# yjpark1/multiagent_rl

Hardware: AMD Instinct MI355X
Metric: env-steps/sec, simple_spread N=6 x B envs, 1/2/4/8 MI355X (higher is better)
Workload: dtype f32

## Files before the change

multiagent_rl_amd/csrc/pw_kernels_spread_quad.hpp:

```cpp
#pragma once

#include "pw_kernels_spread.hpp"

namespace {

__device__ __forceinline__ void quad_pair_of(const int q, int &i, int &j)
{
    i = q < 5 ? 0 : q < 9 ? 1 : q < 12 ? 2 : q < 14 ? 3 : 4;
    j = q - (i == 0 ? 0 : i == 1 ? 5 : i == 2 ? 9 : i == 3 ? 12 : 14) + i + 1;
}

#ifndef PW_QUAD_BARRIER
#define PW_QUAD_BARRIER(t) duo_barrier()
#endif
#ifndef PW_QUAD_ACT_AHEAD
#define PW_QUAD_ACT_AHEAD 4
#endif
constexpr int kQuadActAhead = PW_QUAD_ACT_AHEAD;
constexpr int kQuadActRingBytes = kQuadActAhead * kWave * (int)sizeof(int32_t);
template <bool UNIT_MASS, bool COLL = false, bool K1 = false>
__global__ void __launch_bounds__(4 * kWave) pw_spread_quad_kernel(const StreamParams A, const int T)
{
    constexpr int N = 6, L = 6, D = 16, P2 = 15, EPP = 4, EPW = 8;
    extern __shared__ __attribute__((aligned(16))) unsigned char smem_raw[];
    float4 *s_ring = reinterpret_cast<float4 *>(smem_raw);
    float2 *s_ftab = reinterpret_cast<float2 *>(s_ring + 4 * kWave);
    float *s_min = reinterpret_cast<float *>(s_ftab + 2 * EPP * N * N);
    float *s_rew = s_min + kWave;
    float2 *s_lmB = reinterpret_cast<float2 *>(s_rew + kWave);
    int32_t *s_act = reinterpret_cast<int32_t *>(s_lmB + EPW * L);
    float2 *s_utab = reinterpret_cast<float2 *>(s_act + 2 * kQuadActAhead * kWave);

    const int wave = __builtin_amdgcn_readfirstlane((((int)threadIdx.x >> 6) + 2 * (((int)blockIdx.x >> 8) & 1)) & 3);
    const int lane = (int)threadIdx.x & 63;
    const int env0 = (int)blockIdx.x * EPW;
    const int envs_here = A.B - env0 < EPW ? A.B - env0 : EPW;
    const size_t BN = (size_t)A.B * N;

    const bool resets = A.auto_reset && A.max_episode_len > 0;
    int offs_all = A.ep_step[env0 + (lane < envs_here ? lane : 0)];
    auto next_reset_step = [&](int t_from) -> int {
        if (!resets) return 0x7fffffff;
        int rem = A.max_episode_len - 1 - (t_from + offs_all);
        rem = rem < 0 ? 0 : rem;
        int m = 0x7fffffff;
        for (int e = 0; e < envs_here; ++e) {
            const int r = __builtin_amdgcn_readlane(rem, e);
            m = r < m ? r : m;
        }
        return t_from + m;
    };
    int t_reset = next_reset_step(0);
    auto reset_step_update = [&](int t) {
        if (t + 1 + offs_all >= A.max_episode_len) offs_all = -(t + 1);
        t_reset = next_reset_step(t + 1);
    };
    int cur = 0;

    if (wave < 2) {
        __builtin_amdgcn_s_setprio(3);
        const int e0 = wave * EPP;
        const int nv = envs_here - e0 < 0 ? 0 : envs_here - e0 < EPP ? envs_here - e0 : EPP;
        if (nv == 0) {
            for (int t = 0; t < T; ++t) PW_QUAD_BARRIER(t);
            return;
        }
        const int la = lane < nv * N ? lane : 0;
        const int e4 = la / N, a = la - e4 * N;
        const int me = (e0 + e4) * N + a;
        const int env = env0 + e0 + e4;
        const uint32_t g = (uint32_t)env * (uint32_t)N + (uint32_t)a;
        const uint64_t env_id = A.env_id_base + (uint64_t)env;
        const int lp = lane < nv * P2 ? lane : 0;
        const int pe = lp / P2, pq = lp - pe * P2;
        int pi, pj;
        quad_pair_of(pq, pi, pj);
        const int ri = (e0 + pe) * N + pi, rj = (e0 + pe) * N + pj;
        float2 *ftab = s_ftab + wave * (EPP * N * N);
        float2 *f_ij = ftab + (pe * N + pi) * N + (pj - 1), *f_ji = ftab + (pe * N + pj) * N + pi;
        const float2 *row = ftab + (e4 * N + a) * N;

        float px = A.pos_x[g], py = A.pos_y[g], vx = A.vel_x[g], vy = A.vel_y[g];
        int ep_off = A.ep_step[env];
        uint32_t ep_count = A.ep_count[env];
        s_ring[me] = make_float4(px, py, vx, vy);
        float2 *utab = s_utab + wave * 8;
        if (lane < 6) {
            const int ai = lane;
            float ux = 0.0f + ((ai == 1 ? 1.0f : 0.0f) - (ai == 2 ? 1.0f : 0.0f));
            float uy = 0.0f + ((ai == 3 ? 1.0f : 0.0f) - (ai == 4 ? 1.0f : 0.0f));
            ux *= A.sens; uy *= A.sens;
            if (A.fscale != 1.0f) { ux = A.fscale * ux; uy = A.fscale * uy; }
            utab[lane] = make_float2(ux + 0.0f, uy + 0.0f);
        }
        wave_lds_sync();
        const float k = A.contact_margin, cf = A.contact_force, dt = A.dt, damp = A.damp, mass = A.mass;
        const uint32_t near_lo = __float_as_uint(A.near_thr2), near_span = 0x7F800000u - near_lo;
        const int32_t *act_g = A.act + g;
        int32_t *act_ring = s_act + wave * (kQuadActAhead * kWave);
        const uint32_t act_lds = __builtin_amdgcn_readfirstlane((uint32_t)reinterpret_cast<uintptr_t>(act_ring));
        auto fetch_act = [&](int t) {
            act_fetch_issue(act_g + (size_t)(t < T ? t : T - 1) * BN, act_lds + (uint32_t)(t & (kQuadActAhead - 1)) * (kWave * 4));
        };
        asm volatile("" :: "v"(ep_off), "v"(ep_count), "v"(offs_all), "v"(px), "v"(py), "v"(vx), "v"(vy), "s"(t_reset));
        for (int t0 = 0; t0 < kQuadActAhead; ++t0) fetch_act(t0);
        float2 qi = *reinterpret_cast<const float2 *>(s_ring + ri);
        float2 qj = *reinterpret_cast<const float2 *>(s_ring + rj);
        PW_STAMP_DECL;
        for (int t = 0; t < T; ++t) {
            PW_STAMP_START;
            asm volatile("s_waitcnt vmcnt(%0)" :: "n"(kQuadActAhead - 1) : "memory");
            PW_STAMP(3);
            const uint32_t ai = (uint32_t)act_ring[(t & (kQuadActAhead - 1)) * kWave + lane];
            fetch_act(t + kQuadActAhead);
            const float2 u0 = utab[ai < 5u ? ai : 5u];
            const bool two_slots = t == t_reset;
            float Fx = 0.0f, Fy = 0.0f;
            {
                const float dx = qi.x - qj.x, dy = qi.y - qj.y;
                const float d2 = dx * dx + dy * dy;
                if (__float_as_uint(d2) - near_lo >= near_span)
                    collision_force_pair<true, K1>(qi.x, qi.y, qj.x, qj.y, A.dist_min, k, cf, Fx, Fy);
            }
            *f_ij = make_float2(Fx, Fy);
            *f_ji = make_float2(-Fx, -Fy);
            PW_STAMP(0);
            float fx = u0.x, fy = u0.y;
            asm volatile("" ::: "memory");
#pragma unroll
            for (int j = 0; j < N - 1; ++j) {
                const float2 F = row[j];
                fx = F.x + fx;
                fy = F.y + fy;
            }
            vx = vx * damp; vy = vy * damp;
            vx = vx + div_mass<UNIT_MASS>(fx, mass) * dt;
            vy = vy + div_mass<UNIT_MASS>(fy, mass) * dt;
            px = px + vx * dt;
            py = py + vy * dt;
            int nxt = (cur + 1) & 3;
            s_ring[nxt * kWave + me] = make_float4(px, py, vx, vy);
            if (two_slots) {
                if (t + 1 + ep_off >= A.max_episode_len) {
                    ep_count += 1;
                    ep_off = -(t + 1);
                    pw_reset_xy(A.seed, env_id, ep_count, (uint32_t)a, -1.0f, 1.0f, &px, &py);
                    vx = 0.f; vy = 0.f;
                }
                reset_step_update(t);
                nxt = (nxt + 1) & 3;
                s_ring[nxt * kWave + me] = make_float4(px, py, vx, vy);
            }
            cur = nxt;
            asm volatile("" ::: "memory");
            qi = *reinterpret_cast<const float2 *>(s_ring + cur * kWave + ri);
            qj = *reinterpret_cast<const float2 *>(s_ring + cur * kWave + rj);
            PW_STAMP(1);
            PW_QUAD_BARRIER(t);
            PW_STAMP(2);
        }
        act_fetch_drain();
#ifdef PW_STAMPS
        if (blockIdx.x == 0 && wave == 0 && lane == 0)
            for (int i_ = 0; i_ < 4; ++i_) g_pw_stamps[i_] = st_acc[i_];
#endif
        A.pos_x[g] = px; A.pos_y[g] = py;
        A.vel_x[g] = vx; A.vel_y[g] = vy;
        A.ep_step[env] = T + ep_off;
        A.ep_count[env] = ep_count;
        return;
    }

    int e_local = lane / N;
    int a = lane - e_local * N;
    if (e_local >= envs_here) { e_local = 0; a = 0; }
    const int env = env0 + e_local;
    const int base = e_local * N, me = base + a;
    const uint32_t g = (uint32_t)env * (uint32_t)N + (uint32_t)a;
    const uint64_t env_id = A.env_id_base + (uint64_t)env;
    int ep_off = A.ep_step[env];
    uint32_t ep_count = A.ep_count[env];
    float olx = A.lm_x[(size_t)env * L + a], oly = A.lm_y[(size_t)env * L + a];

    if (wave == 2) {
        float own_p = 0.0f;
        int cnt_p = 0;
        uint32_t cmask_p = 0;
        float2 mine, q6[N];
        auto a_reads = [&](const int nxt) __attribute__((always_inline)) {
            const float4 *slot = s_ring + nxt * kWave + base;
            mine = *reinterpret_cast<const float2 *>(slot + a);
#pragma unroll
            for (int j = 0; j < N; ++j) q6[j] = *reinterpret_cast<const float2 *>(slot + j);
        };
        float best, e0;
        int cnt;
        uint32_t cmask;
        auto a_dist = [&]() __attribute__((always_inline)) {
            const float px = mine.x, py = mine.y;
            float e2[N];
            cnt = 0; cmask = 0;
#pragma unroll
            for (int j = 0; j < N; ++j) {
                const float2 q = q6[j];
                const float dx = q.x - px, dy = q.y - py;
                const float d2 = dx * dx + dy * dy;
                cnt += d2 < A.coll_thr2 ? 1 : 0;
                if (COLL) cmask |= d2 < A.coll_thr2 ? 1u << j : 0u;
                const float ex = q.x - olx, ey = q.y - oly;
                e2[j] = ex * ex + ey * ey;
            }
            best = __builtin_fminf(__builtin_fminf(__builtin_fminf(e2[0], e2[1]), __builtin_fminf(e2[2], e2[3])),
                                   __builtin_fminf(e2[4], e2[5]));
            e0 = e2[0];
        };
        auto a_sqrt = [&]() __attribute__((always_inline)) -> float {
            const float b = e0 != e0 ? e0 : best;
            return sqrtf(b);
        };
        auto a_clock = [&](const int t, int nxt) __attribute__((always_inline)) {
            if (t == t_reset) {
                if (t + 1 + ep_off >= A.max_episode_len) {
                    ep_count += 1;
                    ep_off = -(t + 1);
                    pw_reset_xy(A.seed, env_id, ep_count, (uint32_t)(N + a), -1.0f, 1.0f, &olx, &oly);
                }
                reset_step_update(t);
                nxt = (nxt + 1) & 3;
            }
            cur = nxt;
        };
        float sh_own[L], sh_r[N], r;
        auto b_shfl_own = [&]() __attribute__((always_inline)) {
#pragma unroll
            for (int l = 0; l < L; ++l) sh_own[l] = __shfl(own_p, base + l, kWave);
        };
        auto b_reward = [&]() __attribute__((always_inline)) {
            r = 0.0f;
#pragma unroll
            for (int l = 0; l < L; ++l) r -= sh_own[l];
#pragma unroll
            for (int k2 = 0; k2 < N; ++k2) r -= k2 < cnt_p ? 1.0f : 0.0f;
#pragma unroll
            for (int i = 0; i < N; ++i) sh_r[i] = __shfl(r, base + i, kWave);
        };
        auto b_store = [&](const int tb) __attribute__((always_inline)) {
            const size_t tBN = (size_t)tb * BN;
            float acc = 0.0f;
#pragma unroll
            for (int i = 0; i < N; ++i) acc += sh_r[i];
            nt_store(A.rew + tBN + g, r);
            nt_store(A.rew_shared + (size_t)tb * A.B + env, acc);
            if (COLL) nt_store(A.coll + tBN + g, (uint64_t)cmask_p);
        };
        PW_STAMP_DECL;
        {
            PW_STAMP_START;
            PW_QUAD_BARRIER(0);
            PW_STAMP(0);
            const int nxt = (cur + 1) & 3;
            a_reads(nxt);
            a_dist();
            own_p = a_sqrt(); cnt_p = cnt; cmask_p = cmask;
            a_clock(0, nxt);
            PW_STAMP(1);
        }
        for (int t = 1; t < T; ++t) {
            PW_STAMP_START;
            PW_QUAD_BARRIER(t);
            PW_STAMP(0);
            const int nxt = (cur + 1) & 3;
            a_reads(nxt);
            b_shfl_own();
            a_dist();
            b_reward();
            const float own = a_sqrt();
            b_store(t - 1);
            own_p = own; cnt_p = cnt; cmask_p = cmask;
            a_clock(t, nxt);
            PW_STAMP(1);
        }
        b_shfl_own();
        b_reward();
        b_store(T - 1);
#ifdef PW_STAMPS
        if (blockIdx.x == 0 && lane == 0)
            for (int i_ = 0; i_ < 2; ++i_) g_pw_stamps[4 + i_] = st_acc[i_];
#endif
        return;
    }

    const int rows_here = envs_here * N;
    const int cgrp = lane & 3;
    int row_u[3];
    bool ok_u[3];
#pragma unroll
    for (int u = 0; u < 3; ++u) {
        const int r = (lane >> 2) + 16 * u;
        ok_u[u] = r < rows_here;
        row_u[u] = ok_u[u] ? r : 0;
    }
    float4 lm_u[3];
    auto load_landmarks = [&]() {
#pragma unroll
        for (int u = 0; u < 3; ++u)
            lm_u[u] = *reinterpret_cast<const float4 *>(s_lmB + (row_u[u] / N) * L + (cgrp > 0 ? 2 * cgrp - 2 : 0));
    };
    s_lmB[me] = make_float2(olx, oly);
    wave_lds_sync();
    load_landmarks();
    float4 *const blk4 = reinterpret_cast<float4 *>(A.obs + ((size_t)env0 * N) * D) + lane;
    PW_STAMP_DECL;
    for (int t = 0; t < T; ++t) {
        const size_t tBN = (size_t)t * BN;
        PW_STAMP_START;
        nt_store(A.done + tBN + g, (uint8_t)0);
        PW_QUAD_BARRIER(t);
        PW_STAMP(0);
        int nxt = (cur + 1) & 3;
        nt_store(A.terminal + (size_t)t * A.B + env, (uint8_t)(A.max_episode_len > 0 && t + 1 + ep_off >= A.max_episode_len ? 1 : 0));
        if (t == t_reset) {
            const bool rst = t + 1 + ep_off >= A.max_episode_len;
            if (rst) {
                if (A.final_obs) {
                    const float4 st = s_ring[nxt * kWave + me];
                    stream_write_obs<L>(A.final_obs + (tBN + g) * D, L, s_lmB + base, st.x, st.y, st.z, st.w);
                }
                ep_count += 1;
                ep_off = -(t + 1);
                pw_reset_xy(A.seed, env_id, ep_count, (uint32_t)(N + a), -1.0f, 1.0f, &olx, &oly);
            }
            reset_step_update(t);
            wave_lds_sync();
            if (rst) s_lmB[me] = make_float2(olx, oly);
            wave_lds_sync();
            load_landmarks();
            nxt = (nxt + 1) & 3;
        }
        cur = nxt;
        const float4 *slot = s_ring + nxt * kWave;
        float4 *const out4 = blk4 + tBN * (D / 4);
#pragma unroll
        for (int u = 0; u < 3; ++u) {
            const float4 st = slot[row_u[u]];
            const float4 o = cgrp == 0 ? make_float4(st.z, st.w, st.x, st.y)
                                       : make_float4(lm_u[u].x - st.x, lm_u[u].y - st.y, lm_u[u].z - st.x, lm_u[u].w - st.y);
            if (ok_u[u]) nt_store(out4 + 64 * u, o);
        }
        PW_STAMP(1);
    }
#ifdef PW_STAMPS
    if (blockIdx.x == 0 && lane == 0)
        for (int i_ = 0; i_ < 2; ++i_) g_pw_stamps[6 + i_] = st_acc[i_];
#endif
    A.lm_x[(size_t)env * L + a] = olx;
    A.lm_y[(size_t)env * L + a] = oly;
}

}
```

Measured before the change: 7.600 billion.

## Add fast-path pair force, pointer-bumped stores, custom act fetch in quad kernel

```diff
diff --git a/multiagent_rl_amd/csrc/pw_kernels_spread_quad.hpp b/multiagent_rl_amd/csrc/pw_kernels_spread_quad.hpp
--- a/multiagent_rl_amd/csrc/pw_kernels_spread_quad.hpp
+++ b/multiagent_rl_amd/csrc/pw_kernels_spread_quad.hpp
@@ -10,11 +10,56 @@
     j = q - (i == 0 ? 0 : i == 1 ? 5 : i == 2 ? 9 : i == 3 ? 12 : 14) + i + 1;
 }
 
+__device__ __forceinline__ void quad_act_fetch(const int32_t *row, const uint32_t lane_off, const uint32_t lds_slot, const uint32_t slot_read)
+{
+    unsigned keep;
+    asm volatile("s_mov_b32 %0, m0\n\ts_mov_b32 m0, %3\n\ts_nop 0\n\tglobal_load_lds_dword %1, %2\n\ts_mov_b32 m0, %0"
+                 : "=&s"(keep) : "v"(lane_off), "s"(row), "s"(lds_slot), "v"(slot_read) : "memory");
+}
+
+template <bool K1>
+__device__ __forceinline__ void quad_pair_force(const float2 qi, const float2 qj, const uint32_t near_lo, const uint32_t near_span,
+                                                const float dist_min, const float k, const float cf, float &Fx, float &Fy)
+{
+    const float dx = qi.x - qj.x, dy = qi.y - qj.y;
+    const float d2 = dx * dx + dy * dy;
+    const f32x2 a = {cf * dx, cf * dy};
+    const bool near = __float_as_uint(d2) - near_lo >= near_span;
+    const bool uni = (k >= 9.094947017729282e-13f) & (k <= 1099511627776.0f) & (cf >= 9.5367431640625e-07f) & (cf <= 128.0f);
+    const bool c1 = (__float_as_uint(d2) - 0x12800000u) < (0x6C800000u - 0x12800000u);
+    const bool c2 = fminf(fabsf(a.x), fabsf(a.y)) >= 8.673617379884035e-19f;
+    const bool fast = near & c1 & c2 & uni;
+    const bool any_cold = __builtin_amdgcn_ballot_w64(near & !fast) != 0;
+    Fx = 0.0f; Fy = 0.0f;
+    if (fast) {
+        const float dist = sqrt_rn_core(d2);
+        const float y0 = __builtin_amdgcn_rcpf(dist);
+        __builtin_amdgcn_sched_barrier(0);
+        const float yd = __builtin_fmaf(__builtin_fmaf(-dist, y0, 1.0f), y0, y0);
+        const f32x2 Q = div_chain2(a, dist, yd);
+        const float xarg = K1 ? div_chain1(-(dist - dist_min), k, div_refined_rcp(k))
+                              : div_chain(-(dist - dist_min), k, div_refined_rcp(k));
+        const float pen = softplus_branchless(xarg) * k;
+        const f32x2 F = Q * f32x2{pen, pen};
+        Fx = F.x;
+        Fy = F.y;
+    }
+    if (__builtin_expect(any_cold, 0)) {
+        if (near & !fast) collision_force_pair<true, K1>(qi.x, qi.y, qj.x, qj.y, dist_min, k, cf, Fx, Fy);
+    }
+}
+
 #ifndef PW_QUAD_BARRIER
 #define PW_QUAD_BARRIER(t) duo_barrier()
 #endif
 #ifndef PW_QUAD_ACT_AHEAD
 #define PW_QUAD_ACT_AHEAD 4
+#endif
+#ifndef PW_QUAD_PAD_P
+#define PW_QUAD_PAD_P()
+#endif
+#ifndef PW_QUAD_PAD_OB
+#define PW_QUAD_PAD_OB()
 #endif
 constexpr int kQuadActAhead = PW_QUAD_ACT_AHEAD;
 constexpr int kQuadActRingBytes = kQuadActAhead * kWave * (int)sizeof(int32_t);
@@ -96,14 +141,17 @@
         wave_lds_sync();
         const float k = A.contact_margin, cf = A.contact_force, dt = A.dt, damp = A.damp, mass = A.mass;
         const uint32_t near_lo = __float_as_uint(A.near_thr2), near_span = 0x7F800000u - near_lo;
-        const int32_t *act_g = A.act + g;
+        const unsigned char *act_row = reinterpret_cast<const unsigned char *>(A.act);
+        const size_t act_stride = BN * sizeof(int32_t);
+        const uint32_t act_off = g * (uint32_t)sizeof(int32_t);
         int32_t *act_ring = s_act + wave * (kQuadActAhead * kWave);
         const uint32_t act_lds = __builtin_amdgcn_readfirstlane((uint32_t)reinterpret_cast<uintptr_t>(act_ring));
-        auto fetch_act = [&](int t) {
-            act_fetch_issue(act_g + (size_t)(t < T ? t : T - 1) * BN, act_lds + (uint32_t)(t & (kQuadActAhead - 1)) * (kWave * 4));
+        auto fetch_act = [&](int t, uint32_t slot_read) {
+            quad_act_fetch(reinterpret_cast<const int32_t *>(act_row), act_off, act_lds + (uint32_t)(t & (kQuadActAhead - 1)) * (kWave * 4), slot_read);
+            act_row += t + 1 < T ? act_stride : (size_t)0;
         };
         asm volatile("" :: "v"(ep_off), "v"(ep_count), "v"(offs_all), "v"(px), "v"(py), "v"(vx), "v"(vy), "s"(t_reset));
-        for (int t0 = 0; t0 < kQuadActAhead; ++t0) fetch_act(t0);
+        for (int t0 = 0; t0 < kQuadActAhead; ++t0) fetch_act(t0, 0u);
         float2 qi = *reinterpret_cast<const float2 *>(s_ring + ri);
         float2 qj = *reinterpret_cast<const float2 *>(s_ring + rj);
         PW_STAMP_DECL;
@@ -112,16 +160,11 @@
             asm volatile("s_waitcnt vmcnt(%0)" :: "n"(kQuadActAhead - 1) : "memory");
             PW_STAMP(3);
             const uint32_t ai = (uint32_t)act_ring[(t & (kQuadActAhead - 1)) * kWave + lane];
-            fetch_act(t + kQuadActAhead);
+            fetch_act(t + kQuadActAhead, ai);
             const float2 u0 = utab[ai < 5u ? ai : 5u];
             const bool two_slots = t == t_reset;
-            float Fx = 0.0f, Fy = 0.0f;
-            {
-                const float dx = qi.x - qj.x, dy = qi.y - qj.y;
-                const float d2 = dx * dx + dy * dy;
-                if (__float_as_uint(d2) - near_lo >= near_span)
-                    collision_force_pair<true, K1>(qi.x, qi.y, qj.x, qj.y, A.dist_min, k, cf, Fx, Fy);
-            }
+            float Fx, Fy;
+            quad_pair_force<K1>(qi, qj, near_lo, near_span, A.dist_min, k, cf, Fx, Fy);
             *f_ij = make_float2(Fx, Fy);
             *f_ji = make_float2(-Fx, -Fy);
             PW_STAMP(0);
@@ -140,7 +183,7 @@
             py = py + vy * dt;
             int nxt = (cur + 1) & 3;
             s_ring[nxt * kWave + me] = make_float4(px, py, vx, vy);
-            if (two_slots) {
+            if (__builtin_expect(two_slots, 0)) {
                 if (t + 1 + ep_off >= A.max_episode_len) {
                     ep_count += 1;
                     ep_off = -(t + 1);
@@ -156,6 +199,7 @@
             qi = *reinterpret_cast<const float2 *>(s_ring + cur * kWave + ri);
             qj = *reinterpret_cast<const float2 *>(s_ring + cur * kWave + rj);
             PW_STAMP(1);
+            PW_QUAD_PAD_P();
             PW_QUAD_BARRIER(t);
             PW_STAMP(2);
         }
@@ -219,7 +263,7 @@
             return sqrtf(b);
         };
         auto a_clock = [&](const int t, int nxt) __attribute__((always_inline)) {
-            if (t == t_reset) {
+            if (__builtin_expect(t == t_reset, 0)) {
                 if (t + 1 + ep_off >= A.max_episode_len) {
                     ep_count += 1;
                     ep_off = -(t + 1);
@@ -244,14 +288,17 @@
 #pragma unroll
             for (int i = 0; i < N; ++i) sh_r[i] = __shfl(r, base + i, kWave);
         };
-        auto b_store = [&](const int tb) __attribute__((always_inline)) {
-            const size_t tBN = (size_t)tb * BN;
+        float *rew_t = A.rew, *rsh_t = A.rew_shared;
+        uint64_t *coll_t = A.coll;
+        auto b_store = [&]() __attribute__((always_inline)) {
             float acc = 0.0f;
 #pragma unroll
             for (int i = 0; i < N; ++i) acc += sh_r[i];
-            nt_store(A.rew + tBN + g, r);
-            nt_store(A.rew_shared + (size_t)tb * A.B + env, acc);
-            if (COLL) nt_store(A.coll + tBN + g, (uint64_t)cmask_p);
+            nt_store(rew_t + g, r);
+            nt_store(rsh_t + env, acc);
+            if (COLL) nt_store(coll_t + g, (uint64_t)cmask_p);
+            rew_t += BN; rsh_t += A.B;
+            if (COLL) coll_t += BN;
         };
         PW_STAMP_DECL;
         {
@@ -275,14 +322,14 @@
             a_dist();
             b_reward();
             const float own = a_sqrt();
-            b_store(t - 1);
+            b_store();
             own_p = own; cnt_p = cnt; cmask_p = cmask;
             a_clock(t, nxt);
             PW_STAMP(1);
         }
         b_shfl_own();
         b_reward();
-        b_store(T - 1);
+        b_store();
 #ifdef PW_STAMPS
         if (blockIdx.x == 0 && lane == 0)
             for (int i_ = 0; i_ < 2; ++i_) g_pw_stamps[4 + i_] = st_acc[i_];
@@ -292,13 +339,15 @@
 
     const int rows_here = envs_here * N;
     const int cgrp = lane & 3;
+    const bool col0 = cgrp == 0;
     int row_u[3];
-    bool ok_u[3];
+    uint32_t off_u[3];
 #pragma unroll
     for (int u = 0; u < 3; ++u) {
         const int r = (lane >> 2) + 16 * u;
-        ok_u[u] = r < rows_here;
-        row_u[u] = ok_u[u] ? r : 0;
+        const bool ok = r < rows_here;
+        row_u[u] = ok ? r : 0;
+        off_u[u] = (uint32_t)(ok ? lane + 64 * u : cgrp) * 16u;
     }
     float4 lm_u[3];
     auto load_landmarks = [&]() {
@@ -309,25 +358,29 @@
     s_lmB[me] = make_float2(olx, oly);
     wave_lds_sync();
     load_landmarks();
-    float4 *const blk4 = reinterpret_cast<float4 *>(A.obs + ((size_t)env0 * N) * D) + lane;
+    unsigned char *obs_t = reinterpret_cast<unsigned char *>(A.obs + ((size_t)env0 * N) * D);
+    uint8_t *done_t = A.done, *term_t = A.terminal;
+    const size_t obs_stride = BN * D * sizeof(float);
+    const bool has_len = A.max_episode_len > 0;
+    int t_term = has_len ? A.max_episode_len - 1 - ep_off : 0x7fffffff;
     PW_STAMP_DECL;
     for (int t = 0; t < T; ++t) {
-        const size_t tBN = (size_t)t * BN;
         PW_STAMP_START;
-        nt_store(A.done + tBN + g, (uint8_t)0);
+        nt_store(done_t + g, (uint8_t)0);
         PW_QUAD_BARRIER(t);
         PW_STAMP(0);
         int nxt = (cur + 1) & 3;
-        nt_store(A.terminal + (size_t)t * A.B + env, (uint8_t)(A.max_episode_len > 0 && t + 1 + ep_off >= A.max_episode_len ? 1 : 0));
+        nt_store(term_t + env, (uint8_t)(t >= t_term ? 1 : 0));
         if (t == t_reset) {
-            const bool rst = t + 1 + ep_off >= A.max_episode_len;
+            const bool rst = t >= t_term;
             if (rst) {
                 if (A.final_obs) {
                     const float4 st = s_ring[nxt * kWave + me];
-                    stream_write_obs<L>(A.final_obs + (tBN + g) * D, L, s_lmB + base, st.x, st.y, st.z, st.w);
+                    stream_write_obs<L>(A.final_obs + ((size_t)t * BN + g) * D, L, s_lmB + base, st.x, st.y, st.z, st.w);
                 }
                 ep_count += 1;
                 ep_off = -(t + 1);
+                t_term = A.max_episode_len - 1 - ep_off;
                 pw_reset_xy(A.seed, env_id, ep_count, (uint32_t)(N + a), -1.0f, 1.0f, &olx, &oly);
             }
             reset_step_update(t);
@@ -339,14 +392,19 @@
         }
         cur = nxt;
         const float4 *slot = s_ring + nxt * kWave;
-        float4 *const out4 = blk4 + tBN * (D / 4);
+        float4 st[3];
+#pragma unroll
+        for (int u = 0; u < 3; ++u) st[u] = slot[row_u[u]];
+        asm volatile("" :: "v"(st[0].x), "v"(st[0].y), "v"(st[0].z), "v"(st[0].w), "v"(st[1].x), "v"(st[1].y), "v"(st[1].z),
+                           "v"(st[1].w), "v"(st[2].x), "v"(st[2].y), "v"(st[2].z), "v"(st[2].w));
 #pragma unroll
         for (int u = 0; u < 3; ++u) {
-            const float4 st = slot[row_u[u]];
-            const float4 o = cgrp == 0 ? make_float4(st.z, st.w, st.x, st.y)
-                                       : make_float4(lm_u[u].x - st.x, lm_u[u].y - st.y, lm_u[u].z - st.x, lm_u[u].w - st.y);
-            if (ok_u[u]) nt_store(out4 + 64 * u, o);
-        }
+            const float4 d = make_float4(lm_u[u].x - st[u].x, lm_u[u].y - st[u].y, lm_u[u].z - st[u].x, lm_u[u].w - st[u].y);
+            const float4 o = make_float4(col0 ? st[u].z : d.x, col0 ? st[u].w : d.y, col0 ? st[u].x : d.z, col0 ? st[u].y : d.w);
+            nt_store(reinterpret_cast<float4 *>(obs_t + off_u[u]), o);
+        }
+        obs_t += obs_stride; done_t += BN; term_t += A.B;
+        PW_QUAD_PAD_OB();
         PW_STAMP(1);
     }
 #ifdef PW_STAMPS
```

Measured after the change: 7.814 billion (median of 6 runs). 2.8% higher.
